# instadeepai/FrameDiPT

Measured on AMD Instinct MI355X. Metric: residue*diffusion-steps/sec, higher is better.
Workload: dtype fp16

## Files before the change

### framedipt_amd/csrc/model.hip

```cpp
#include <math.h>
#include <string.h>

#include <vector>

#include "common.hpp"
#include "kernels.hpp"

struct LinW { long w, b; int out, in; };
struct LNW { long g, b; int d; };
#define FD_MAX_BLOCKS 8
#define FD_MAX_TL 4
struct TfLayer { LinW inp, outp, l1, l2; LNW n1, n2; };
struct BlockW {
  long head_w;
  LinW q, kv, qp, kvp, lb, dz, out, rbf;
  LNW ipa_ln;
  LinW skip;
  TfLayer tf[FD_MAX_TL];
  LinW post, t1, t2, t3;
  LNW tln;
  LinW bb;
  LinW et_init, et1, et2, etf;
  LNW et_ln;
};
// ... 542 lines not shown
  w.pz = take(use_regpair(d) ? fd_pz_bytes(B, N) : 0);
  w.ee_tab = take(ee_table_static(d, B, N) ? fd_ee2_table_bytes(B, ee_table_max_rel(N), d->num_bins) : 0);
  w.ee_idx = take(ee_table_static(d, B, N) ? NN * 4 : 0);
  w.ee_lead = take((size_t)B * 4);
  w.total = o;
}

size_t fdipt_forward_workspace_bytes(const FdiptDims* dims, int B, int N) {
  if (!dims_ok(dims) || B <= 0 || N <= 0) return 0;
  Inventory iv;
  DLayout L;
  WS w;
  build_inventory(dims, iv);
  blob_walk(dims, iv, L);
  build_ws(dims, iv, L, B, N, w);
  return w.total;
}

}

enum { OP_ALL, OP_EMBED, OP_POINTS, OP_IPA, OP_ET };
struct OpSel {
  int kind = OP_ALL, block = 0;
  const float* node_in = nullptr;
  const void* z_in = nullptr;
  void* z_out = nullptr;
  float* node_out = nullptr;
  float* out = nullptr;
  float *qp = nullptr, *kp = nullptr, *vp = nullptr;
};

enum NodeForm { NF_GEMM, NF_ROWBLOCK, NF_ROWS16 };
enum SkipAt { SKIP_PER_BLOCK, SKIP_EMBED16, SKIP_SPLITK };
enum OutProj { OUT_GEMM, OUT_DEDICATED, OUT_SPLITK_SPLIT };
enum NodeRows { NR_PROJ, NR_POINTS, NR_LAUNCH };
enum SeqAttn { SEQ_FUSED, SEQ_BF16, SEQ_F32, SEQ_GENERIC };
enum PostAt { POST_TAIL, POST_CHAIN, POST_GEMM };
enum EtKind { ET_GEMM, ET_CHAIN, ET_ET3, ET_ET4 };
enum EtRows { ETR_IMAGES, ETR_ROWS, ETR_FOLDED };
struct ForwardPlan {
  int op;
  bool bf, fused_node;
  NodeForm embed, tail, transition, torsion;
  SkipAt skip;
  OutProj outproj;
  int slices;
// ... 112 lines not shown
  size_t NN;
  const float* res_mask = a->res_mask;
  float* F(size_t off) const { return (float*)(W + off); }
  FdStep step() const { return FdStep{a->step_cursor, a->frame_rows, a->state_ring}; }
  const void* WM(const LinW& l) const { return p.bf ? (const void*)((const half_t*)(D + L.h16_base) + l.w) : (const void*)(P + l.w); }
  int lin(const LinW& l, const float* A, int lda, const float* res, int ldr, const float* rm, int relu, float* out, int ldo) const {
    return fd_linear(op_precision(d), R, l.out, l.in, A, lda, WM(l), l.in, P + l.b, res, ldr, rm, relu, out, ldo, st);
  }
  int lin32(const LinW& l, const float* A, int lda, float* out, int ldo) const {
    return fd_linear(FDIPT_PREC_F32, R, l.out, l.in, A, lda, P + l.w, l.in, P + l.b, nullptr, 0, nullptr, 0, out, ldo, st);
  }
  int d2d(void* dst, const void* src, size_t bytes) const {
    return hipMemcpyAsync(dst, src, bytes, hipMemcpyDeviceToDevice, st) == hipSuccess ? FDIPT_OK : FDIPT_ELAUNCH;
  }
  int inner(int b, int slot, const float* src, int ld, int cols) const {
    if (!a->trace_inner) return FDIPT_OK;
    float* dst = a->trace_inner + ((size_t)(b * 4 + slot) * R) * iv.d_t;
    return hipMemcpy2DAsync(dst, (size_t)iv.d_t * 4, src, (size_t)ld * 4, (size_t)cols * 4, R, hipMemcpyDeviceToDevice, st) == hipSuccess
               ? FDIPT_OK : FDIPT_ELAUNCH;
  }
  bool first_block(int b) const { return b == 0 || p.op != OP_ALL; }
  bool bias_ready(int b) const { return p.op == OP_ALL && (b == 0 ? p.ee_bias : (p.et == ET_ET3 || p.et == ET_ET4) && p.et_bias); }
  bool fold_et_rows(int b) const { return p.et_rows == ETR_FOLDED && b < d->num_blocks - 1; }
  L2Warm warm_of(int b, WarmOf next, int l = 0) const {
    const DBlock& db = L.blk[b];
    const int cs = d->c_s, dt = iv.d_t;
    const unsigned tb = (unsigned)fd_chain_image_bytes(cs, cs);
    switch (next) {
      case WARM_QKV: {
        const unsigned n = (unsigned)fd_chain_image_bytes(3 * dt, dt);
        return L2Warm{{D + db.ch.inp[l], D + db.lo.inp[l], nullptr}, {n, n, 0}};
      }
      case WARM_TAIL: {
        if (p.tail == NF_ROWS16) return L2Warm{{D + db.lo.o16[l][0], D + db.lo.o16[l][1], nullptr}, {db.lo.tail16_run[l], db.lo.tail16_run[l], 0}};
        const unsigned wimg = (unsigned)fd_chain_image_bytes(dt, dt);
        return L2Warm{{D + db.ch.outp[l], D + db.ch.l1[l], D + db.ch.l2[l]}, {wimg, wimg, wimg}};
      }
      case WARM_POST: return L2Warm{{D + db.ch.post, nullptr, nullptr}, {(unsigned)fd_chain_image_bytes(cs, dt), 0, 0}};
      case WARM_TRANSITION:
        if (p.transition == NF_ROWS16) return L2Warm{{D + db.lo.tr16[0][0], D + db.lo.tr16[0][1], nullptr}, {db.lo.tr16_run, db.lo.tr16_run, 0}};
        return L2Warm{{D + db.ch.t1, D + db.ch.t2, D + db.lo.t1}, {tb, db.ch.t23_run, db.lo.t_run}};
      case WARM_TRANSITION32:
        return L2Warm{{D + db.ch.t1, D + db.ch.t2, D + db.ch.t3}, {tb, tb, tb}};
      case WARM_ET_ROWS: {
        const unsigned ei = (unsigned)fd_chain_image_bytes(iv.cb, cs), r4 = (unsigned)fd_chain_image_bytes(2 * (iv.hid + d->c_z), iv.cb);
        return L2Warm{{D + db.ch.et_init, D + db.ch.r4w, D + db.lo.et_init}, {ei, r4, db.lo.et_run}};
      }
      case WARM_ET_FOLDED:
        return L2Warm{{D + db.lo.ei16[0], D + db.lo.ei16[1], nullptr}, {db.lo.et16_run, db.lo.et16_run, 0}};
      case WARM_TORSION:
        if (p.torsion == NF_ROWS16) return L2Warm{{D + L.tor16[0][0], D + L.tor16[0][1], nullptr}, {L.tor16_run, L.tor16_run, 0}};
        return L2Warm{{D + L.ch_tor1, D + L.ch_tor2, D + L.lo_tor1}, {tb, tb, L.lo_tor_run}};
    }
    return L2Warm{};
  }
  int embed_stage() const {
    const int cs = d->c_s, cz = d->c_z;
    RC(fd_build_feats(B, N, d->use_aatype, d->index_embed, a->aatype, a->t_emb, a->t_emb_eps, a->fixed_mask, a->idx_emb, F(w.node_feat),
                      L.kn_pad, F(w.pte), L.d1_pad, p.feats_fused ? a->rigids_t : nullptr, a->res_mask, d->coordinate_scaling, F(w.quat),
                      F(w.trans), F(w.dmask), (const float*)(D + L.w1i), (const float*)(D + L.w1j), (const float*)(D + L.b1), cz,
                      p.feats_fused ? F(w.pi) : nullptr, F(w.pj), step(), st));
    if (p.embed == NF_GEMM) {
      RC(fd_linear(op_precision(d), R, cs, L.kn_pad, F(w.node_feat), L.kn_pad, D + L.ne0_pad, L.kn_pad, P + iv.ne0.b, nullptr, 0, nullptr, 1,
                   F(w.h_a), cs, st));
      RC(lin(iv.ne2, F(w.h_a), cs, nullptr, 0, nullptr, 1, F(w.h_b), cs));
      RC(lin(iv.ne4, F(w.h_b), cs, nullptr, 0, nullptr, 0, F(w.h_a), cs));
      RC(fd_layernorm(R, cs, F(w.h_a), cs, nullptr, 0, P + iv.neln.g, P + iv.neln.b, a->res_mask, F(w.node0), cs, st));
    } else {
      const bool r16 = p.embed == NF_ROWS16;
      RowBlockArgs r;
      r.M = R; r.in = F(w.node_feat); r.ld_in = L.kn_pad;
      r.w0 = D + (r16 ? L.ne16[0][0] : L.ch_ne0); r.w1 = D + (r16 ? L.ne16[1][0] : L.ch_ne2); r.w2 = D + (r16 ? L.ne16[2][0] : L.ch_ne4);
      r.w0l = D + (r16 ? L.ne16[0][1] : L.lo_ne0); r.w1l = D + (r16 ? L.ne16[1][1] : L.lo_ne2); r.w2l = D + (r16 ? L.ne16[2][1] : L.lo_ne4);
      r.b0 = P + iv.ne0.b; r.b1 = P + iv.ne2.b; r.b2 = P + iv.ne4.b;
      r.gamma = P + iv.neln.g; r.beta = P + iv.neln.b; r.rowmask_post = a->res_mask; r.out = F(w.node0); r.ld_out = cs;
      if (p.skip == SKIP_EMBED16) {
        r.w3 = D + L.skip16[0]; r.w3l = D + L.skip16[1]; r.b3 = (const float*)(D + L.skip_b);
        r.out2 = F(w.skip_all); r.ld_out2 = d->num_blocks * d->c_skip;
        r.warm = L2Warm{{r.w0, r.w0l, r.w3}, {L.ne16_run, L.ne16_run, L.skip16_run}};
      }
      if (r16) RC(fd_node_embed16(r, L.kn_pad, st));
      else RC(fd_rowblock(L.kn_pad == 72 ? FD_RB_NODE_EMBED_72 : FD_RB_NODE_EMBED_88, r, st));
    }
    if (!p.feats_fused) {
      RC(fd_linear(FDIPT_PREC_F32, R, cz, L.d1_pad, F(w.pte), L.d1_pad, D + L.w1i, L.d1_pad, (const float*)(D + L.b1), nullptr, 0,
                   nullptr, 0, F(w.pi), cz, st));
      RC(fd_linear(FDIPT_PREC_F32, R, cz, L.d1_pad, F(w.pte), L.d1_pad, D + L.w1j, L.d1_pad, nullptr, nullptr, 0, nullptr, 0,
                   F(w.pj), cz, st));
    }
    EdgeEmbedArgs ea;
    ea.B = B; ea.N = N; ea.n_rel = a->n_rel; ea.rel_off = a->rel_off; ea.num_bins = d->num_bins;
    ea.pi = F(w.pi); ea.pj = F(w.pj); ea.rtab = (const float*)setup; ea.dtab = d->num_bins > 0 ? (const float*)(D + L.dtab) : nullptr;
    ea.edges = d->num_bins > 0 ? (const float*)(D + L.edges) : nullptr; ea.seq_idx = a->seq_idx; ea.sc_ca = a->sc_ca_t;
    ea.w2 = WM(iv.ee2); ea.w3 = WM(iv.ee4); ea.b2 = P + iv.ee2.b; ea.b3 = P + iv.ee4.b;
    ea.gamma = P + iv.eeln.g; ea.beta = P + iv.eeln.b; ea.res_mask = a->res_mask; ea.z_out = W + w.z;
    ea.trace = a->trace_edge; ea.reserve_cus = a->reserve_cus;
    ea.wb_img = p.ee_bias ? D + L.blk[0].wb_img4 : nullptr; ea.bb = (const float*)(D + L.blk[0].bb); ea.bias_out = F(w.bias); ea.H = d->no_heads;
    if (p.pz) {
      ea.wdz_img = D + L.blk[0].wdz_imgp; ea.wdz_img_lo = D + L.blk[0].wdz_imgp_lo; ea.bdz = P + iv.blk[0].dz.b; ea.pz_out = (half_t*)(W + w.pz);
    }
    if (p.ee_table) {
      ea.fixed_mask = a->fixed_mask; ea.table = W + w.ee_tab; ea.row_idx = (int32_t*)(W + w.ee_idx); ea.leaders = (int32_t*)(W + w.ee_lead);
      ea.rel_lead = (const int32_t*)((const char*)setup + setup_rel_lead(d, B, a->n_rel));
      RC(fd_edge_embed2_leaders(ea, st));
      RC(fd_edge_embed2_table(ea, D + (p.x ? L.ee2x : L.ee2), st, p.x));
      ea.pz_out = nullptr;
      RC(fd_edge_embed2_spread(ea, st, 0));
    } else if (p.regpair) RC(fd_edge_embed2(ea, D + (p.x ? L.ee2x : L.ee2), st, p.x));
    else RC(fd_edge_embed(op_precision(d), cz, ea, st));
    return FDIPT_OK;
  }
  int ipa_project(int b, const float* node) const {
    const DBlock& db = L.blk[b];
    const int cs = d->c_s, H = d->no_heads, C = d->c_hidden, Pq = d->no_qk_points, Pv = d->no_v_points, PT = iv.proj_out - 3 * H * C;
    PointsArgs pa;
    pa.B = B; pa.N = N; pa.H = H; pa.Pq = Pq; pa.Pv = Pv; pa.quat = F(w.quat); pa.trans = F(w.trans);
    pa.qp = F(w.qp); pa.kp = F(w.kp); pa.vp = F(w.vp); pa.rot = F(w.rot);
    pa.vpt = p.vpt ? (unsigned short*)(W + w.vpt) : nullptr; pa.Np = Np;
    if (!p.a3) {
      RC(fd_linear(op_precision(d), R, iv.proj_out, cs, node, cs, D + db.wproj, cs, (const float*)(D + db.bproj), nullptr, 0,
                   nullptr, 0, F(w.proj), iv.proj_out, st));
      pa.proj = F(w.proj); pa.ld = iv.proj_out; pa.q_off = 3 * H * C; pa.kv_off = 3 * H * C + 3 * H * Pq;
      return fd_points(pa, st);
    }
    pa.kpf = (unsigned short*)(W + w.kpf); pa.gamma = (const float*)(D + db.gamma); pa.res_mask = a->res_mask;
    ProjArgs pj;
    pj.B = B; pj.N = N; pj.H = H; pj.C = C; pj.K = cs; pj.PT = PT; pj.Np = Np; pj.A = node; pj.lda = cs;
    pj.W = D + db.wproj; pj.bias = (const float*)(D + db.bproj); pj.qscale = sqrtf(1.0f / (3.0f * (float)C));
    pj.Qb = (half_t*)(W + w.qb); pj.Kb = (half_t*)(W + w.kb); pj.Vt = (half_t*)(W + w.vt); pj.pts = F(w.pts);
    pj.zero_pads = first_block(b);
    pj.W_img = proj_image(d) ? D + db.wproj_img : nullptr;
    pj.W_img_lo = pj.W_img && p.fused_node ? D + db.wproj_img_lo : nullptr;
    if (p.merged) { pj.merged = 1; pj.W_img = D + db.wproj2_img; pj.W_img_lo = D + db.wproj2_img_lo; pj.bias = (const float*)(D + db.bproj2); }
    if (p.proj_pts) {
      pj.pts_img = 1; pj.W_img = D + db.wproj2p_img; pj.W_img_lo = D + db.wproj2p_img_lo; pj.bias = (const float*)(D + db.bproj2p);
      pj.PT = fd_ipa_proj2_points_cols(H, C) - H * C;
      pj.quat = pa.quat; pj.trans = pa.trans; pj.gamma = pa.gamma; pj.res_mask = pa.res_mask; pj.rot = pa.rot; pj.qp = pa.qp;
      pj.kpf = pa.kpf; pj.vpt = pa.vpt;
    }
    if (p.vt_lo && p.node_rows == NR_PROJ) pj.Vt_lo = (half_t*)(W + w.vt_lo);
    const size_t vpt_bytes = (size_t)B * H * 96 * Np * 2;
    bool vpt_zero = pa.vpt && first_block(b);
    if (p.proj2) {
      const bool key_pads = Np > N && p.node_rows == NR_PROJ;
      if (pj.zero_pads && p.init_fused) {
        SeqInitExtra sx = {vpt_zero ? W + w.vpt : nullptr, vpt_zero ? (long)(vpt_bytes >> 4) : 0L, key_pads ? (void*)pj.Kb : nullptr,
                           (void*)pj.Vt, (long)B * H, C, (void*)pj.Vt_lo};
        RC(fd_seq_images_init(B, N, d->tfmr_heads, a->res_mask, W + w.seqimg, sx, st, p.stream));
        vpt_zero = false;
      } else if (pj.zero_pads && (key_pads || vpt_zero)) {
        ProjArgs pz = pj; pz.W_img = nullptr;
        if (p.node_rows != NR_PROJ) pz.Np = pz.N;
        RC(fd_ipa_proj_zero_pads(pz, vpt_zero ? W + w.vpt : nullptr, vpt_zero ? vpt_bytes : 0, st));
        vpt_zero = false;
      }
      RC(fd_ipa_proj2(pj, st));
      half_t* vt_lo = (half_t*)(W + w.vt_lo);
      if (p.node_rows == NR_POINTS) { pa.node = node; pa.ld_node = cs; pa.nKb = pj.Kb; pa.nVt = pj.Vt; pa.nVt_lo = vt_lo; }
      if (p.node_rows == NR_LAUNCH) RC(fd_node_images(B, N, Np, node, cs, pj.Kb, pj.Vt, vt_lo, st));
    } else RC(fd_ipa_proj(pj, st));
    if (vpt_zero && hipMemsetAsync(W + w.vpt, 0, vpt_bytes, st) != hipSuccess) return FDIPT_ELAUNCH;
    pa.proj = F(w.pts); pa.ld = PT; pa.q_off = 0; pa.kv_off = 3 * H * Pq;
    if (!p.proj_pts) RC(fd_points(pa, st));
    return FDIPT_OK;
  }
  int ipa_attend(int b) const {
    const DBlock& db = L.blk[b];
    const int cz = d->c_z, H = d->no_heads, C = d->c_hidden, Pv = d->no_v_points, feat = iv.feat_dim;
    OPairArgs oa;
    oa.B = B; oa.N = N; oa.H = H; oa.CZ = cz; oa.CD = cz / 4; oa.z = W + w.z; oa.probs = F(w.probs); oa.probs_h16 = nullptr;
    oa.probs_np = 0; oa.out_h16 = nullptr; oa.wdz = (const float*)(D + db.wdz_t); oa.wdz_img = p.bf && dz_images(d) ? D + db.wdz_img : nullptr;
// ... 255 lines not shown
    if (!setup || !a->fixed_mask || (!a->sc_ca_t && d->num_bins > 0) || !a->seq_idx || !a->idx_emb || !a->t_emb) return FDIPT_EINVAL;
    if (d->use_aatype && (!a->aatype || !a->t_emb_eps)) return FDIPT_EINVAL;
  }
  if (op.kind == OP_ALL && (!a->rigids_t || !a->gt_psi || !a->t || !a->so3_sigma || !a->psi || !a->rot_score || !a->trans_score ||
                            !a->rigids))
    return FDIPT_EINVAL;
  if ((op.kind == OP_POINTS || op.kind == OP_IPA) && !a->rigids_t) return FDIPT_EINVAL;
  if (!FdStep{a->step_cursor, a->frame_rows, a->state_ring}.valid()) return FDIPT_EINVAL;
  if (op.kind != OP_ALL && op.kind != OP_EMBED && (op.block < 0 || op.block >= d->num_blocks - (op.kind == OP_ET ? 1 : 0))) return FDIPT_EINVAL;
  Inventory iv;
  DLayout L;
  WS w;
  build_inventory(d, iv);
  blob_walk(d, iv, L);
  const int B = a->B, N = a->N, R = B * N;
  build_ws(d, iv, L, B, N, w);
  if (workspace_bytes < w.total) return FDIPT_ESIZE;
  if ((long)B * N * N > 2000000000L / 1) return FDIPT_ESIZE;
  const ForwardPlan p = plan_forward(d, iv, L, B, N, op.kind, a->n_rel, a->trace_edge != nullptr, a->pair_embed != 0);
  if (p.refused) return FDIPT_EINVAL;
  const Fwd f = {d, iv, L, w, p, P, (const char*)derived, (char*)workspace, setup, a, (hipStream_t)stream, B, N, R, (N + 31) / 32 * 32, (size_t)R * N};
  if (a->trace_inner && (p.fused_node || p.outproj != OUT_GEMM)) return FDIPT_EINVAL;
  const size_t node_bytes = (size_t)R * d->c_s * 4, z_bytes = f.NN * d->c_z * L.esz;
  if (op.kind == OP_ALL || op.kind == OP_EMBED) RC(f.embed_stage());
  if (op.kind == OP_EMBED) {
    if (op.node_out) RC(f.d2d(op.node_out, f.F(w.node0), node_bytes));
    if (op.z_out) RC(f.d2d(op.z_out, f.W + w.z, z_bytes));
    return FDIPT_OK;
  }
  if (a->trace_node && op.kind == OP_ALL) RC(f.d2d(a->trace_node, f.F(w.node0), node_bytes));
  if (!p.feats_fused && a->rigids_t)
    RC(fd_split_rigids(R, a->rigids_t, d->coordinate_scaling, a->res_mask, a->fixed_mask ? a->fixed_mask : a->res_mask, f.F(w.quat),
                       f.F(w.trans), f.F(w.dmask), f.step(), f.st));
  if (op.kind != OP_ALL) {
    if (!op.node_in) return FDIPT_EINVAL;
    RC(f.d2d(f.F(w.node), op.node_in, node_bytes));
    if (op.kind != OP_POINTS) {
      if (!op.z_in) return FDIPT_EINVAL;
      RC(f.d2d(f.W + w.z, op.z_in, z_bytes));
    }
    const int b = op.block;
    if (op.kind == OP_ET) {
      RC(f.edge_transition_stage(b, f.F(w.node)));
      if (!op.z_out) return FDIPT_EINVAL;
      return f.d2d(op.z_out, f.W + w.z, z_bytes);
    }
// ... 39 lines not shown
  build_inventory(d, iv);
  blob_walk(d, iv, L);
  const ForwardPlan p = plan_forward(d, iv, L, B, N, OP_ALL, n_rel, false, false);
  return p.ee_table && !p.refused ? (int64_t)n_rel * (d->num_bins + 1) : 0;
}

int fdipt_embed_table_leaders(const FdiptDims* d, const void* workspace, int B, int N, int n_rel, int32_t* out_dev) {
  if (!workspace || !out_dev || fdipt_embed_table_rows(d, B, N, n_rel) <= 0) return FDIPT_EINVAL;
  Inventory iv;
  DLayout L;
  WS w;
  build_inventory(d, iv);
  blob_walk(d, iv, L);
  build_ws(d, iv, L, B, N, w);
  if (hipDeviceSynchronize() != hipSuccess) return FDIPT_ELAUNCH;
  return hipMemcpy(out_dev, (const char*)workspace + w.ee_lead, (size_t)B * 4, hipMemcpyDeviceToDevice) == hipSuccess ? FDIPT_OK : FDIPT_ELAUNCH;
}

int fdipt_score_forward(const FdiptDims* d, const float* P, const void* derived, const void* setup,
                        const FdiptForwardArgs* a, void* workspace, size_t workspace_bytes, fdipt_stream_t stream) {
  return forward_impl(d, P, derived, setup, a, workspace, workspace_bytes, stream, OpSel{});
}

int fdipt_edge_embed_fwd(const FdiptDims* d, const float* P, const void* derived, const void* setup, const FdiptForwardArgs* a,
                         float* node_out, void* z_out, void* workspace, size_t workspace_bytes, fdipt_stream_t stream) {
  OpSel op;
  op.kind = OP_EMBED; op.node_out = node_out; op.z_out = z_out;
  return forward_impl(d, P, derived, setup, a, workspace, workspace_bytes, stream, op);
}

static FdiptForwardArgs op_args(int B, int N, const float* rigids_t, const float* res_mask) {
  FdiptForwardArgs a;
  memset(&a, 0, sizeof(a));
  a.B = B; a.N = N; a.rigids_t = rigids_t; a.res_mask = res_mask;
  return a;
}
int fdipt_ipa_project_points(const FdiptDims* d, const float* P, const void* derived, int block, int B, int N, const float* node,
                             const float* rigids, const float* res_mask, float* q_pts, float* k_pts, float* v_pts,
                             void* workspace, size_t workspace_bytes, fdipt_stream_t stream) {
  OpSel op;
  op.kind = OP_POINTS; op.block = block; op.node_in = node; op.qp = q_pts; op.kp = k_pts; op.vp = v_pts;
  const FdiptForwardArgs a = op_args(B, N, rigids, res_mask);
  return forward_impl(d, P, derived, nullptr, &a, workspace, workspace_bytes, stream, op);
}
int fdipt_ipa_attention_fwd(const FdiptDims* d, const float* P, const void* derived, int block, int B, int N, const float* node,
                            const void* z, const float* rigids, const float* res_mask, float* out, void* workspace,
// ... 34 lines not shown
```

### framedipt_amd/inference.py

```python
from __future__ import annotations

import ctypes as C

import numpy as np
import torch

from . import _lib, gpu_guard
from . import noise as noise_mod
from .model.score_network import preprocess_aatype


def draw_noise_tape(diffuser, n_steps: int, B: int, N: int):
    z_rot = np.zeros((n_steps, B, N, 3))
    z_trans = np.zeros((n_steps, B, N, 3))
    for s in range(n_steps):
        if diffuser._diffuse_rot:
            z_rot[s] = np.random.normal(size=(B, N, 3))
        if diffuser._diffuse_trans:
            z_trans[s] = np.random.normal(size=(B, N, 3))
    return z_rot, z_trans


def kept_steps(num_t: int, keep="all") -> np.ndarray:
    num_t = int(num_t)
# ... 27 lines not shown
    _lib.check(lib.fdipt_backbone_atoms(n, _lib.ptr(t7), _lib.ptr(rot), _lib.ptr(trans), _lib.ptr(psi), _lib.ptr(aatype),
                                        _lib.ptr(net.bb_tables), _lib.ptr(atom37), None, _lib.stream_ptr()),
               "backbone_atoms")


def get_atom_positions_from_rigids(model, rigids, psi_torsions, aatype=None) -> np.ndarray:
    t7 = rigids.to_tensor_7() if hasattr(rigids, "to_tensor_7") else rigids
    dev = model.device
    with torch.cuda.device(dev):
        t7 = t7.to(device=dev, dtype=torch.float32).contiguous()
        psi = psi_torsions.to(device=dev, dtype=torch.float32).contiguous()
        aa = None if aatype is None else aatype.to(device=dev, dtype=torch.int32).contiguous()
        atom37 = torch.empty(t7.shape[:-1] + (37, 3), dtype=torch.float32, device=dev)
        _backbone(model, int(np.prod(t7.shape[:-1])), t7, None, None, psi, aa, atom37)
        return atom37.cpu().numpy()


class ReverseLoop:

    GRAPH_CHUNK = 8

    def __init__(self, model, diffuser, data_init, num_t, min_t, center=True, aux_traj=False, self_condition=True,
                 noise_scale=1.0, embed_self_conditioning=True, inpainting=False, input_aatype=False, noise_tape=None, state=None,
                 graph=True, verify=0, noise="host", noise_keys=None, keep="all"):
        self.model, self.diffuser = model, diffuser
        self.keep = keep
        steps = kept_steps(num_t, keep)
        self.kept = keep != "all"
        keys = noise_mod.resolve(noise, noise_keys, noise_tape, int(data_init["rigids_t"].shape[0]))
        dev = self.dev = model.device
        gpu_guard.check(dev, what="inference_fn")
        self.verify, self.verified = int(verify or 0), 0
        rig0 = data_init["rigids_t"]
        _lib.require_cuda(rig0, "inference_fn")
        if rig0.dim() == 2:
            raise ValueError("rigids_t needs a leading batch dimension")
        B, N = self.B, self.N = rig0.shape[0], rig0.shape[1]
        f32 = lambda x: x.to(device=dev, dtype=torch.float32).contiguous().clone()
        self.res_mask, self.fixed = f32(data_init["res_mask"]), f32(data_init["fixed_mask"])
        self.fixed_mask = (self.fixed * self.res_mask).contiguous()
        self.diffuse_mask = ((1 - self.fixed) * self.res_mask).contiguous()
        self._inpainting, self._input_aatype = inpainting, input_aatype
        self.aatype, self.net_aatype, same = _aatype_views(model, data_init, self.fixed, inpainting, input_aatype, dev)
        self.bb0_from_forward = same
        self.gt_tors = data_init["torsion_angles_sin_cos"]
        self.gt_psi = f32(self.gt_tors[..., 2, :])
        self.st = state if state is not None else model.batch_state(data_init["seq_idx"])
        self.num_t, self.min_t, self.dt = num_t, min_t, 1 / num_t
        self.center, self.aux_traj, self.noise_scale = center, aux_traj, noise_scale
        self.self_condition, self.embed_sc = self_condition, embed_self_conditioning
        self.reverse_steps = np.linspace(min_t, 1.0, num_t)[::-1]
        n_noisy = self.n_noisy = int(np.sum(self.reverse_steps > min_t))
        t32, temb, sig = model.step_scalars(self.reverse_steps)
        with torch.cuda.device(dev):
            self.t_all = torch.as_tensor(np.repeat(t32[:, None], B, 1), device=dev)
            self.temb_all = torch.as_tensor(np.repeat(temb[:, None, :], B, 1), device=dev)
            self.sig_all = torch.as_tensor(np.repeat(sig[:, None], B, 1), device=dev)
            self.t_tab = torch.as_tensor(np.ascontiguousarray(self.reverse_steps, dtype=np.float64), device=dev)
            so3 = diffuser._so3_diffuser
            self.tab_all = self.omega_edges = None
            if so3.use_cached_score:
                rows = so3.score_table_rows(t32)
                self.tab_all = torch.as_tensor(np.repeat(rows[:, None, :], B, 1), device=dev)
                self.omega_edges = torch.as_tensor(so3.omega_edges, device=dev)
            self.z_rot = self.z_trans = self.noise_keys = None
            if keys is not None:
                self.noise_keys = noise_mod.keys_tensor(keys, dev)
            else:
                if noise_tape is None:
                    noise_tape = draw_noise_tape(diffuser, n_noisy, B, N)
                self.z_rot = torch.as_tensor(np.ascontiguousarray(noise_tape[0], dtype=np.float64), device=dev)
                self.z_trans = torch.as_tensor(np.ascontiguousarray(noise_tape[1], dtype=np.float64), device=dev)
            self.sc_ca = f32(data_init["sc_ca_t"])
            self.kept_steps, n_rows = steps, len(steps)
            self.frame_rows = self.kept_rigids = None
            self._row_of = None
# ... 12 lines not shown
            self.trans_traj = torch.empty(n_rows, B, N, 3, device=dev) if aux_traj else None
            self.cursor = torch.zeros(2, dtype=torch.int32, device=dev)
        self.graph = bool(graph) and n_noisy >= 3 and (keys is not None or (self.z_rot.shape[0] >= n_noisy and self.z_trans.shape[0] >= n_noisy))
        self._cursor_host = 0
        self._g1 = self._gn = None
        self.capture_seconds = 0.0
        self.captures = 0

    @property
    def rigids_t(self):
        return self._x(self._next)

    _next = 0

    def _x(self, k):
        return self.rigid_traj[k & 1] if self.kept else self.rigid_traj[k]

    def _row(self, k):
        if not self.kept:
            return k
        r = int(self._row_of[k])
        return None if r < 0 else r

    def _fwd(self, k, want_atoms, sc_update):
        row = self._row(k)
        want_atoms = want_atoms and row is not None
        direct = want_atoms and self.bb0_from_forward
        self.st.score_table = None if self.tab_all is None else self.tab_all[k]
        self.st.omega_edges = self.omega_edges
        self.st.forward(self._x(k), self.res_mask, self.fixed, self.sc_ca, self.net_aatype, self.gt_psi, self.t_all[k],
                        self.temb_all[k], self.sig_all[k], direct, ca_out=self.sc_ca if sc_update else None,
                        atom37_out=self.bb0_traj[row] if direct else None)
        if want_atoms and not direct:
            _backbone(self.model, self.B * self.N, self.st.rigids, None, None, self.st.psi, self.aatype, self.bb0_traj[row])

    def prime(self):
        if self.embed_sc and self.self_condition:
            with torch.cuda.device(self.dev):
                self._fwd(0, False, True)

    def _verify_forward(self, k):
        st = self.st
        self.st.score_table = None if self.tab_all is None else self.tab_all[k]
        self.st.omega_edges = self.omega_edges
        st.forward(self._x(k), self.res_mask, self.fixed, self.sc_ca, self.net_aatype, self.gt_psi, self.t_all[k],
                   self.temb_all[k], self.sig_all[k], False)
        return [x.clone() for x in (st.rigids, st.psi, st.rot_score, st.trans_score)]

    def _step_eager(self, k):
        st, t, n = self.st, self.reverse_steps[k], self.B * self.N
        first = self._verify_forward(k) if self.verify and k % self.verify == 0 else None
        self._fwd(k, self.aux_traj, self.embed_sc and t > self.min_t)
        if first is not None:
            for name, a, b in zip(("rigids", "psi", "rot_score", "trans_score"), first, (st.rigids, st.psi, st.rot_score, st.trans_score)):
                if not torch.equal(a, b):
                    raise _lib.FdiptError(f"verify: two runs of the forward of step {k} differ in `{name}` (max |diff| "
                                          f"{float((a - b).abs().max()):.3e}): results on this GPU are not reproducible — is another "
                                          "compute process using it? (DESIGN.md section 6)")
            self.verified += 1
        nxt, row = self._x(k + 1), self._row(k)
        if t > self.min_t:
            dev_noise = self.noise_keys is not None
            self.diffuser.reverse_device(self._x(k), st.rot_score, st.trans_score, self.diffuse_mask,
                                         None if dev_noise else self.z_rot[k], None if dev_noise else self.z_trans[k], t, self.dt,
                                         self.center, self.noise_scale, rigids_out=nxt, noise_keys=self.noise_keys, step=k,
                                         atoms=(st.psi, self.aatype, self.model.bb_tables, self.prot_traj[row]) if row is not None else None,
                                         traj=(st.rigids, self.fixed_mask, self.trans_traj[row]) if self.aux_traj and row is not None else None)
        else:
            nxt.copy_(st.rigids)
            _backbone(self.model, n, nxt, None, None, st.psi, self.aatype, self.prot_traj[row])
            if self.aux_traj:
                self.trans_traj[row] = self.diffuse_mask[..., None] * st.rigids[..., 4:] + self.fixed_mask[..., None] * nxt[..., 4:]
        if self.kept_rigids is not None and row is not None:
            self.kept_rigids[row].copy_(nxt)

    def _enqueue_indexed(self):
        lib, st, d = _lib.load(), self.st, self.diffuser
        direct = self.aux_traj and self.bb0_from_forward
        st.score_table, st.omega_edges = self.tab_all, self.omega_edges
        st.forward(self.rigid_traj, self.res_mask, self.fixed, self.sc_ca, self.net_aatype, self.gt_psi, self.t_all, self.temb_all,
                   self.sig_all, direct, ca_out=self.sc_ca if self.embed_sc else None, atom37_out=self.bb0_traj if direct else None,
                   step_cursor=self.cursor, frame_rows=self.frame_rows, state_ring=self.kept)
        if self.aux_traj and not direct:
            args = [self.B * self.N, _lib.ptr(st.rigids), _lib.ptr(st.psi), _lib.ptr(self.aatype), _lib.ptr(self.model.bb_tables),
                    _lib.ptr(self.bb0_traj), _lib.ptr(self.cursor)]
            if self.kept:
                _lib.check(lib.fdipt_backbone_atoms_kept(*args, _lib.ptr(self.frame_rows), _lib.stream_ptr()), "backbone_atoms_kept")
            else:
                _lib.check(lib.fdipt_backbone_atoms_indexed(*args, _lib.stream_ptr()), "backbone_atoms_indexed")
        so3, r3 = d._so3_diffuser, d._r3_diffuser
        a = _lib.ReverseIndexed()
        a.B, a.N = self.B, self.N
        for name, tns in (("rigid_traj", self.rigid_traj), ("rot_score", st.rot_score), ("trans_score", st.trans_score),
                          ("diffuse_mask", self.diffuse_mask), ("z_rot", self.z_rot), ("z_trans", self.z_trans), ("t_table", self.t_tab),
                          ("psi", st.psi), ("aatype", self.aatype), ("bb_tables", self.model.bb_tables), ("prot_traj", self.prot_traj),
                          ("pred_rigids", st.rigids if self.aux_traj else None), ("traj_fixed_mask", self.fixed_mask if self.aux_traj else None),
                          ("trans_traj", self.trans_traj), ("step_cursor", self.cursor), ("frame_rows", self.frame_rows),
                          ("kept_rigids", self.kept_rigids)):
            setattr(a, name, _lib.ptr(tns))
        a.state_ring = int(self.kept)
        a.dt, a.noise_scale = float(self.dt), float(self.noise_scale)
        a.center, a.diffuse_rot, a.diffuse_trans = int(bool(self.center)), int(bool(d._diffuse_rot)), int(bool(d._diffuse_trans))
        a.so3_min_sigma, a.so3_max_sigma, a.r3_min_b, a.r3_max_b = so3.min_sigma, so3.max_sigma, r3.min_b, r3.max_b
        a.coordinate_scaling = r3._r3_conf.coordinate_scaling
        if self.noise_keys is not None:
# ... 24 lines not shown
            self.cursor[:1].fill_(k)
            self._cursor_host = k

    _WARM: set = set()

    def _warm_key(self):
        return (str(self.dev), bytes(self.model.dims), self.B, self.N, bool(self.aux_traj), bool(self.bb0_from_forward),
                bool(self._inpainting), self.tab_all is not None, bool(self.embed_sc), bool(self.self_condition),
                self.noise_keys is not None, bool(self.kept))

    def prepare(self):
        if self.graph and self._warm_key() in self._WARM:
            with torch.cuda.device(self.dev):
                if self._g1 is None:
                    self._g1 = self.capture_step_graph(1)
                if self._gn is None and self.GRAPH_CHUNK > 1 and self.n_noisy >= 2 * self.GRAPH_CHUNK:
                    self._gn = self.capture_step_graph(self.GRAPH_CHUNK)
        return self

    def _advance(self, k, n, eager=False):
        self._set_cursor(k)
        if (self._g1 is not None or self._gn is not None) and self._captured_weights != getattr(self.model, "weights_version", 0):
            self._g1 = self._gn = None
        if eager or self._warm_key() not in self._WARM:
            for _ in range(n):
                self._enqueue_indexed()
            self._WARM.add(self._warm_key())
        elif n > 1 and n == self.GRAPH_CHUNK:
            if self._gn is None:
                self._gn = self.capture_step_graph(n)
            self._gn.replay()
        else:
            if self._g1 is None:
                self._g1 = self.capture_step_graph(1)
            for _ in range(n):
                self._g1.replay()
        self._cursor_host = k + n

    def step(self, k, eager=False):
        with torch.cuda.device(self.dev):
            if self.graph and k < self.n_noisy and not (self.verify and k % self.verify == 0):
                self._advance(k, 1, eager)
            else:
                self._step_eager(k)
        self._next = k + 1

# ... 47 lines not shown
        if self.diffuser._so3_diffuser.use_cached_score != (self.tab_all is not None):
            raise ValueError("reset: so3.use_cached_score changed behind the loop: the score-table switch selects other launches")
        before = self._warm_key()
        with torch.cuda.device(dev):
            f32 = lambda x: x.to(device=dev, dtype=torch.float32).contiguous()
            fixed = f32(data_init["fixed_mask"])
            aatype, net_aatype, same = _aatype_views(self.model, data_init, fixed, self._inpainting, self._input_aatype, dev)
            if same != self.bb0_from_forward or (aatype is None) != (self.aatype is None) or (net_aatype is None) != (self.net_aatype is None):
                raise ValueError("reset: this batch changes who builds the rigid_0_traj rows (bb0_from_forward / the aatype views): the captured "
                                 "launch sequence does not fit it; construct a new loop")
            seq_idx = data_init["seq_idx"]
            if tuple(seq_idx.shape) != (self.B, self.N):
                raise ValueError(f"reset: seq_idx of shape {tuple(seq_idx.shape)}, the loop holds B, N = {self.B}, {self.N}")
            keys = tape = None
            if self.noise_keys is not None:
                keys = noise_mod.keys_tensor(noise_mod.resolve("device", noise_keys, noise_tape, self.B), dev)
            else:
                if noise_tape is None:
                    noise_tape = draw_noise_tape(self.diffuser, self.n_noisy, self.B, self.N)
                tape = [torch.as_tensor(np.ascontiguousarray(z, dtype=np.float64)) for z in noise_tape]
                for dst, z in zip((self.z_rot, self.z_trans), tape):
                    if tuple(z.shape) != tuple(dst.shape):
                        raise ValueError(f"reset: noise tape of shape {tuple(z.shape)}, the loop's is {tuple(dst.shape)}")
            if getattr(self.model, "_state", None) is self.st:
                self.model._state = self.model._state_key = None
            if keys is not None:
                self.noise_keys.copy_(keys)
            else:
                self.z_rot.copy_(tape[0])
                self.z_trans.copy_(tape[1])
            self.res_mask.copy_(f32(data_init["res_mask"]))
            self.fixed.copy_(fixed)
            torch.mul(self.fixed, self.res_mask, out=self.fixed_mask)
            torch.mul(1 - self.fixed, self.res_mask, out=self.diffuse_mask)
            if aatype is not None:
                self.aatype.copy_(aatype)
            if net_aatype is not None:
                self.net_aatype.copy_(net_aatype)
            self.gt_tors = data_init["torsion_angles_sin_cos"]
            self.gt_psi.copy_(f32(self.gt_tors[..., 2, :]))
            self.sc_ca.copy_(f32(data_init["sc_ca_t"]))
            self.rigid_traj[0].copy_(rig0.to(device=dev, dtype=torch.float32))
            if not self.st.refresh(seq_idx):
                self._g1 = self._gn = None
            self.cursor.zero_()
        self._cursor_host, self._next, self.verified = 0, 0, 0
# ... 164 lines not shown
```

### framedipt_amd/model/score_network.py

```python
from __future__ import annotations

import ctypes as C
from collections import OrderedDict

import numpy as np
import torch

from .. import _lib, embedding, residue_tables, weights


PRECISIONS = {"fp32": _lib.PREC_F32, "f32": _lib.PREC_F32, "fp16": _lib.PREC_F16, "f16": _lib.PREC_F16,
              "fp16x": _lib.PREC_F16X, "f16x": _lib.PREC_F16X,
              "bf16": _lib.PREC_BF16}


def dims_from_conf(model_conf, diffuser_conf, inpainting: bool, precision: int, kernel_flags: int = 0) -> _lib.Dims:
    i, e = model_conf.ipa, model_conf.embed
    num_bins = e.num_bins if e.embed_self_conditioning else 0
    return _lib.Dims(i.c_s, i.c_z, i.c_hidden, i.c_skip, i.no_heads, i.no_qk_points, i.no_v_points,
                     i.seq_tfmr_num_heads, i.seq_tfmr_num_layers, i.num_blocks, e.index_embed_size, num_bins,
                     int(bool(inpainting or model_conf.input_aatype)), precision, kernel_flags, float(e.min_bin), float(e.max_bin),
                     float(i.coordinate_scaling), float(diffuser_conf.r3.min_b), float(diffuser_conf.r3.max_b))


# ... 55 lines not shown
    def refresh(self, seq_idx: torch.Tensor) -> bool:
        if tuple(seq_idx.shape) != (self.B, self.N):
            raise ValueError(f"refresh: seq_idx of shape {tuple(seq_idx.shape)}, the state holds B, N = {self.B}, {self.N}")
        lib, net, dev = _lib.load(), self.net, self.net.device
        sidx = seq_idx.detach().cpu().numpy().astype(np.int64)
        if np.array_equal(sidx, self._sidx):
            return True
        self._sidx = sidx
        E, d = net.dims.index_embed, net.dims
        with torch.cuda.device(dev):
            self.seq_idx.copy_(torch.as_tensor(sidx.astype(np.int32)))
            self.idx_emb.copy_(torch.as_tensor(embedding.get_index_embedding(sidx, E)))
            rng = int(sidx.max() - sidx.min())
            if rng == self.rel_off:
                return True
            self.rel_off, self.n_rel = rng, 2 * rng + 1
            rel = np.arange(self.n_rel) - rng
            rel_emb = torch.as_tensor(np.broadcast_to(embedding.get_index_embedding(rel, E)[None], (self.B, self.n_rel, E)).copy(), device=dev)
            self.setup = torch.empty(lib.fdipt_setup_bytes(C.byref(d), self.B, self.N, self.n_rel), dtype=torch.uint8, device=dev)
            _lib.check(lib.fdipt_sample_setup(C.byref(d), _lib.ptr(net.params), _lib.ptr(net.derived), self.B, self.N, self.n_rel,
                                              _lib.ptr(rel_emb), _lib.ptr(self.setup), _lib.stream_ptr()), "sample_setup")
        return False

    def forward(self, rigids_t, res_mask, fixed_mask, sc_ca_t, aatype, gt_psi, t_dev, t_emb_dev, sigma_dev,
                want_atoms: bool = True, ca_out=None, atom37_out=None, step_cursor=None, frame_rows=None, state_ring=False):
        lib = _lib.load()
        net = self.net
        a = _lib.ForwardArgs()
        a.B, a.N, a.n_rel, a.rel_off = self.B, self.N, self.n_rel, self.rel_off
        for name, tns in (("rigids_t", rigids_t), ("res_mask", res_mask), ("fixed_mask", fixed_mask), ("sc_ca_t", sc_ca_t),
                          ("seq_idx", self.seq_idx), ("idx_emb", self.idx_emb), ("aatype", aatype), ("gt_psi", gt_psi),
                          ("t", t_dev), ("t_emb", t_emb_dev), ("t_emb_eps", self.t_emb_eps), ("so3_sigma", sigma_dev),
                          ("bb_tables", net.bb_tables), ("psi", self.psi), ("rot_score", self.rot_score),
                          ("trans_score", self.trans_score), ("rigids", self.rigids),
                          ("atom37", (self.atom37 if atom37_out is None else atom37_out) if want_atoms else None), ("atom14", self.atom14 if want_atoms else None),
                          ("trace_node", self.trace_node), ("trace_edge", self.trace_edge), ("trace_inner", self.trace_inner),
                          ("ca_out", ca_out)):
            setattr(a, name, _lib.ptr(tns))
        if self.ev_start is not None:
            a.ev_start, a.ev_stop = self.ev_start, self.ev_stop
        a.reserve_cus = self.reserve_cus
        a.pair_embed = self.pair_embed
        a.step_cursor = _lib.ptr(step_cursor)
        if step_cursor is not None:
            a.frame_rows, a.state_ring = _lib.ptr(frame_rows), int(bool(state_ring))
        a.clock_out = _lib.ptr(self.clock_out)
        if self.score_table is not None:
            a.so3_score_table, a.so3_omega_edges = _lib.ptr(self.score_table), _lib.ptr(self.omega_edges)
            a.so3_num_omega = int(self.score_table.shape[-1])
        _lib.check(lib.fdipt_score_forward(C.byref(net.dims), _lib.ptr(net.params), _lib.ptr(net.derived),
                                           _lib.ptr(self.setup), C.byref(a), _lib.ptr(self.ws), self.ws_bytes,
                                           _lib.stream_ptr()), "score_forward")


class ScoreNetwork:
    def __init__(self, model_conf, diffuser, inpainting: bool = False, precision: str = "fp32", device=None,
                 kernel_flags: int = 0):
        self._model_conf = model_conf
# ... 119 lines not shown
```

### include/fdipt.h

```cpp
#ifndef FDIPT_H
#define FDIPT_H

#include <stddef.h>
#include <stdint.h>

#ifdef __cplusplus
extern "C" {
#endif

#define FDIPT_OK 0
#define FDIPT_EINVAL (-1)
#define FDIPT_ELAUNCH (-2)
#define FDIPT_ESIZE (-3)

#define FDIPT_PREC_F32 0
#define FDIPT_PREC_BF16 1
#define FDIPT_PREC_F16 2
#define FDIPT_PREC_F16X 3

#define FDIPT_KF_ET3 1
#define FDIPT_KF_GENERIC_PAIR 2
#define FDIPT_KF_GENERIC_ATTN 4
#define FDIPT_KF_UNFUSED_NODE 8
#define FDIPT_KF_UNFOLDED 16
// ... 19 lines not shown
  int32_t num_blocks;
  int32_t index_embed;
  int32_t num_bins;
  int32_t use_aatype;
  int32_t precision;
  int32_t kernel_flags;
  float min_bin;
  float max_bin;
  float coordinate_scaling;
  float r3_min_b;
  float r3_max_b;
} FdiptDims;

int fdipt_param_count(const FdiptDims* dims);
int64_t fdipt_param_offset(const FdiptDims* dims, int index);

size_t fdipt_derived_bytes(const FdiptDims* dims);
int fdipt_model_prepare(const FdiptDims* dims, const float* params_f32, void* derived, fdipt_stream_t stream);

size_t fdipt_setup_bytes(const FdiptDims* dims, int B, int N, int n_rel);
int fdipt_sample_setup(const FdiptDims* dims, const float* params_f32, const void* derived, int B, int N, int n_rel,
                       const float* rel_emb, void* setup, fdipt_stream_t stream);

typedef struct FdiptForwardArgs {
  int32_t B, N, n_rel, rel_off;
  const float* rigids_t;
  const float* res_mask;
  const float* fixed_mask;
  const float* sc_ca_t;
  const int32_t* seq_idx;
  const float* idx_emb;
  const int32_t* aatype;
  const float* gt_psi;
  const float* t;
  const float* t_emb;
  const float* t_emb_eps;
  const double* so3_sigma;
  const void* bb_tables;
  float* psi;
  double* rot_score;
  float* trans_score;
  float* rigids;
  float* atom37;
  float* atom14;
  float* trace_node;
  float* trace_edge;
  float* trace_inner;
  void** ev_start;
  void** ev_stop;
  float* ca_out;
  int32_t reserve_cus;
  int32_t pair_embed;
  unsigned long long* clock_out;
  const double* so3_score_table;
  const double* so3_omega_edges;
  int32_t so3_num_omega;
  const int32_t* step_cursor;
  const int32_t* frame_rows;
  int32_t state_ring;
} FdiptForwardArgs;

size_t fdipt_forward_workspace_bytes(const FdiptDims* dims, int B, int N);
int64_t fdipt_embed_table_rows(const FdiptDims* dims, int B, int N, int n_rel);
int fdipt_embed_table_leaders(const FdiptDims* dims, const void* workspace, int B, int N, int n_rel, int32_t* out_dev);
int fdipt_score_forward(const FdiptDims* dims, const float* params_f32, const void* derived, const void* setup,
                        const FdiptForwardArgs* args, void* workspace, size_t workspace_bytes, fdipt_stream_t stream);

int fdipt_edge_embed_fwd(const FdiptDims* dims, const float* params_f32, const void* derived, const void* setup,
                         const FdiptForwardArgs* args, float* node_out, void* z_out, void* workspace, size_t workspace_bytes,
                         fdipt_stream_t stream);
int fdipt_ipa_project_points(const FdiptDims* dims, const float* params_f32, const void* derived, int block, int B, int N,
                             const float* node, const float* rigids, const float* res_mask, float* q_pts, float* k_pts,
                             float* v_pts, void* workspace, size_t workspace_bytes, fdipt_stream_t stream);
int fdipt_ipa_attention_fwd(const FdiptDims* dims, const float* params_f32, const void* derived, int block, int B, int N,
                            const float* node, const void* z, const float* rigids, const float* res_mask, float* out,
                            void* workspace, size_t workspace_bytes, fdipt_stream_t stream);
int fdipt_edge_transition_fwd(const FdiptDims* dims, const float* params_f32, const void* derived, int block, int B, int N,
                              const float* node, const float* res_mask, const void* z_in, void* z_out, void* workspace,
                              size_t workspace_bytes, fdipt_stream_t stream);

int fdipt_se3_reverse_step(int B, int N, const float* rigids_t, const double* rot_score, const float* trans_score,
                           const float* diffuse_mask , const double* z_rot, const double* z_trans,
                           double t, double dt, double noise_scale, int center, int diffuse_rot, int diffuse_trans,
                           double so3_min_sigma, double so3_max_sigma, double r3_min_b, double r3_max_b,
                           double coordinate_scaling, float* rigids_out , float* out_rot ,
                           fdipt_stream_t stream);
int fdipt_se3_reverse_step_atoms(int B, int N, const float* rigids_t, const double* rot_score, const float* trans_score,
                                 const float* diffuse_mask, const double* z_rot, const double* z_trans, double t, double dt,
                                 double noise_scale, int center, int diffuse_rot, int diffuse_trans, double so3_min_sigma,
// ... 606 lines not shown
```

Measured before the change: 1.231 million.

## Precompute step-invariant edge-table leaders and sequence image pads once per sample

Result: no change. 1.238 million (median of 6 runs) (+0.5%).

```diff
diff --git a/framedipt_amd/csrc/model.hip b/framedipt_amd/csrc/model.hip
--- a/framedipt_amd/csrc/model.hip
+++ b/framedipt_amd/csrc/model.hip
@@ -588,6 +588,7 @@
 enum { OP_ALL, OP_EMBED, OP_POINTS, OP_IPA, OP_ET };
 struct OpSel {
   int kind = OP_ALL, block = 0;
+  bool constants = false;
   const float* node_in = nullptr;
   const void* z_in = nullptr;
   void* z_out = nullptr;
@@ -746,6 +747,11 @@
   bool first_block(int b) const { return b == 0 || p.op != OP_ALL; }
   bool bias_ready(int b) const { return p.op == OP_ALL && (b == 0 ? p.ee_bias : (p.et == ET_ET3 || p.et == ET_ET4) && p.et_bias); }
   bool fold_et_rows(int b) const { return p.et_rows == ETR_FOLDED && b < d->num_blocks - 1; }
+  bool constants_plan() const {
+    return p.op == OP_ALL && p.ee_table && p.a3 && p.seq == SEQ_FUSED && p.init_fused && !p.stream && p.proj_pts && p.node_rows == NR_PROJ && p.vt_lo;
+  }
+  bool pads_kept() const { return constants_plan() && (a->step_constants & FDIPT_SC_PADS); }
+  bool leaders_kept() const { return constants_plan() && (a->step_constants & FDIPT_SC_LEADERS); }
   L2Warm warm_of(int b, WarmOf next, int l = 0) const {
     const DBlock& db = L.blk[b];
     const int cs = d->c_s, dt = iv.d_t;
@@ -778,13 +784,14 @@
     }
     return L2Warm{};
   }
-  int embed_stage() const {
+  int embed_stage(bool leaders_only = false) const {
     const int cs = d->c_s, cz = d->c_z;
     RC(fd_build_feats(B, N, d->use_aatype, d->index_embed, a->aatype, a->t_emb, a->t_emb_eps, a->fixed_mask, a->idx_emb, F(w.node_feat),
                       L.kn_pad, F(w.pte), L.d1_pad, p.feats_fused ? a->rigids_t : nullptr, a->res_mask, d->coordinate_scaling, F(w.quat),
                       F(w.trans), F(w.dmask), (const float*)(D + L.w1i), (const float*)(D + L.w1j), (const float*)(D + L.b1), cz,
                       p.feats_fused ? F(w.pi) : nullptr, F(w.pj), step(), st));
-    if (p.embed == NF_GEMM) {
+    if (leaders_only) {
+    } else if (p.embed == NF_GEMM) {
       RC(fd_linear(op_precision(d), R, cs, L.kn_pad, F(w.node_feat), L.kn_pad, D + L.ne0_pad, L.kn_pad, P + iv.ne0.b, nullptr, 0, nullptr, 1,
                    F(w.h_a), cs, st));
       RC(lin(iv.ne2, F(w.h_a), cs, nullptr, 0, nullptr, 1, F(w.h_b), cs));
@@ -826,13 +833,26 @@
     if (p.ee_table) {
       ea.fixed_mask = a->fixed_mask; ea.table = W + w.ee_tab; ea.row_idx = (int32_t*)(W + w.ee_idx); ea.leaders = (int32_t*)(W + w.ee_lead);
       ea.rel_lead = (const int32_t*)((const char*)setup + setup_rel_lead(d, B, a->n_rel));
-      RC(fd_edge_embed2_leaders(ea, st));
+      if (leaders_only || !leaders_kept()) RC(fd_edge_embed2_leaders(ea, st));
+      if (leaders_only) return FDIPT_OK;
       RC(fd_edge_embed2_table(ea, D + (p.x ? L.ee2x : L.ee2), st, p.x));
       ea.pz_out = nullptr;
       RC(fd_edge_embed2_spread(ea, st, 0));
     } else if (p.regpair) RC(fd_edge_embed2(ea, D + (p.x ? L.ee2x : L.ee2), st, p.x));
     else RC(fd_edge_embed(op_precision(d), cz, ea, st));
     return FDIPT_OK;
+  }
+  int images_init(bool vpt_zero, bool key_pads, bool vt_lo) const {
+    const int H = d->no_heads;
+    const size_t vpt_bytes = (size_t)B * H * 96 * Np * 2;
+    SeqInitExtra sx = {vpt_zero ? W + w.vpt : nullptr, vpt_zero ? (long)(vpt_bytes >> 4) : 0L, key_pads ? (void*)(W + w.kb) : nullptr,
+                       (void*)(W + w.vt), (long)B * H, d->c_hidden, vt_lo ? (void*)(W + w.vt_lo) : nullptr};
+    return fd_seq_images_init(B, N, d->tfmr_heads, a->res_mask, W + w.seqimg, sx, st, p.stream);
+  }
+  int step_constants_stage() const {
+    if (!constants_plan()) return FDIPT_EINVAL;
+    RC(embed_stage(true));
+    return images_init(true, Np > N, true);
   }
   int ipa_project(int b, const float* node) const {
     const DBlock& db = L.blk[b];
@@ -867,10 +887,10 @@
     bool vpt_zero = pa.vpt && first_block(b);
     if (p.proj2) {
       const bool key_pads = Np > N && p.node_rows == NR_PROJ;
-      if (pj.zero_pads && p.init_fused) {
-        SeqInitExtra sx = {vpt_zero ? W + w.vpt : nullptr, vpt_zero ? (long)(vpt_bytes >> 4) : 0L, key_pads ? (void*)pj.Kb : nullptr,
-                           (void*)pj.Vt, (long)B * H, C, (void*)pj.Vt_lo};
-        RC(fd_seq_images_init(B, N, d->tfmr_heads, a->res_mask, W + w.seqimg, sx, st, p.stream));
+      if (pj.zero_pads && pads_kept()) {
+        vpt_zero = false;
+      } else if (pj.zero_pads && p.init_fused) {
+        RC(images_init(vpt_zero, key_pads, pj.Vt_lo != nullptr));
         vpt_zero = false;
       } else if (pj.zero_pads && (key_pads || vpt_zero)) {
         ProjArgs pz = pj; pz.W_img = nullptr;
@@ -1172,6 +1192,7 @@
   const Fwd f = {d, iv, L, w, p, P, (const char*)derived, (char*)workspace, setup, a, (hipStream_t)stream, B, N, R, (N + 31) / 32 * 32, (size_t)R * N};
   if (a->trace_inner && (p.fused_node || p.outproj != OUT_GEMM)) return FDIPT_EINVAL;
   const size_t node_bytes = (size_t)R * d->c_s * 4, z_bytes = f.NN * d->c_z * L.esz;
+  if (op.constants) return f.step_constants_stage();
   if (op.kind == OP_ALL || op.kind == OP_EMBED) RC(f.embed_stage());
   if (op.kind == OP_EMBED) {
     if (op.node_out) RC(f.d2d(op.node_out, f.F(w.node0), node_bytes));
@@ -1257,6 +1278,26 @@
   return forward_impl(d, P, derived, setup, a, workspace, workspace_bytes, stream, OpSel{});
 }
 
+int fdipt_forward_step_constants(const FdiptDims* d, const float* P, const void* derived, const void* setup,
+                                 const FdiptForwardArgs* a, void* workspace, size_t workspace_bytes, fdipt_stream_t stream) {
+  OpSel op;
+  op.constants = true;
+  return forward_impl(d, P, derived, setup, a, workspace, workspace_bytes, stream, op);
+}
+
+int fdipt_forward_image_offsets(const FdiptDims* d, int B, int N, int64_t* offsets_host) {
+  if (!dims_ok(d) || B <= 0 || N <= 0 || !offsets_host) return FDIPT_EINVAL;
+  Inventory iv;
+  DLayout L;
+  WS w;
+  build_inventory(d, iv);
+  blob_walk(d, iv, L);
+  build_ws(d, iv, L, B, N, w);
+  const size_t off[5] = {w.seqimg, w.kb, w.vt, w.vt_lo, w.vpt};
+  for (int i = 0; i < 5; ++i) offsets_host[i] = (int64_t)off[i];
+  return FDIPT_OK;
+}
+
 int fdipt_edge_embed_fwd(const FdiptDims* d, const float* P, const void* derived, const void* setup, const FdiptForwardArgs* a,
                          float* node_out, void* z_out, void* workspace, size_t workspace_bytes, fdipt_stream_t stream) {
   OpSel op;
diff --git a/framedipt_amd/inference.py b/framedipt_amd/inference.py
--- a/framedipt_amd/inference.py
+++ b/framedipt_amd/inference.py
@@ -73,7 +73,7 @@
 
     def __init__(self, model, diffuser, data_init, num_t, min_t, center=True, aux_traj=False, self_condition=True,
                  noise_scale=1.0, embed_self_conditioning=True, inpainting=False, input_aatype=False, noise_tape=None, state=None,
-                 graph=True, verify=0, noise="host", noise_keys=None, keep="all"):
+                 graph=True, verify=0, noise="host", noise_keys=None, keep="all", step_constants=True):
         self.model, self.diffuser = model, diffuser
         self.keep = keep
         steps = kept_steps(num_t, keep)
@@ -103,6 +103,9 @@
         self.reverse_steps = np.linspace(min_t, 1.0, num_t)[::-1]
         n_noisy = self.n_noisy = int(np.sum(self.reverse_steps > min_t))
         t32, temb, sig = model.step_scalars(self.reverse_steps)
+        self._t_host, self._temb_host = np.repeat(t32[:, None], B, 1), np.repeat(temb[:, None, :], B, 1)
+        bits = (_lib.SC_PADS | _lib.SC_LEADERS) if step_constants is True else int(step_constants or 0)
+        self.step_constants = bits if self.st.step_constants_supported() and self.st.uniform_t(self._t_host, self._temb_host) else 0
         with torch.cuda.device(dev):
             self.t_all = torch.as_tensor(np.repeat(t32[:, None], B, 1), device=dev)
             self.temb_all = torch.as_tensor(np.repeat(temb[:, None, :], B, 1), device=dev)
@@ -161,29 +164,55 @@
         r = int(self._row_of[k])
         return None if r < 0 else r
 
+    @property
+    def constants_token(self):
+        tok = self.__dict__.get("_constants_token")
+        if tok is None:
+            tok = self.__dict__["_constants_token"] = object()
+        return tok
+
+    def _ensure_constants(self):
+        if self.step_constants and self.st.constants_owner is not self.constants_token:
+            self.st.write_step_constants(self.constants_token, self.rigid_traj[0], self.res_mask, self.fixed, self.sc_ca, self.net_aatype, self.gt_psi,
+                                         self.t_all[0], self.temb_all[0], self.sig_all[0], self._t_host, self._temb_host)
+
+    def _drop_constants(self):
+        if self.st.constants_owner is self.constants_token:
+            self.st.constants_owner = None
+
+    def _constants(self, k=None):
+        if not self.step_constants:
+            return {}
+        t, temb = (self._t_host, self._temb_host) if k is None else (self._t_host[k], self._temb_host[k])
+        return dict(constants_owner=self.constants_token, constants=self.step_constants, t_host=t, t_emb_host=temb)
+
     def _fwd(self, k, want_atoms, sc_update):
         row = self._row(k)
         want_atoms = want_atoms and row is not None
         direct = want_atoms and self.bb0_from_forward
         self.st.score_table = None if self.tab_all is None else self.tab_all[k]
         self.st.omega_edges = self.omega_edges
+        self._ensure_constants()
         self.st.forward(self._x(k), self.res_mask, self.fixed, self.sc_ca, self.net_aatype, self.gt_psi, self.t_all[k],
                         self.temb_all[k], self.sig_all[k], direct, ca_out=self.sc_ca if sc_update else None,
-                        atom37_out=self.bb0_traj[row] if direct else None)
+                        atom37_out=self.bb0_traj[row] if direct else None,
+                        **self._constants(k))
         if want_atoms and not direct:
             _backbone(self.model, self.B * self.N, self.st.rigids, None, None, self.st.psi, self.aatype, self.bb0_traj[row])
 
     def prime(self):
-        if self.embed_sc and self.self_condition:
-            with torch.cuda.device(self.dev):
+        with torch.cuda.device(self.dev):
+            self._ensure_constants()
+            if self.embed_sc and self.self_condition:
                 self._fwd(0, False, True)
 
     def _verify_forward(self, k):
         st = self.st
         self.st.score_table = None if self.tab_all is None else self.tab_all[k]
         self.st.omega_edges = self.omega_edges
+        self._ensure_constants()
         st.forward(self._x(k), self.res_mask, self.fixed, self.sc_ca, self.net_aatype, self.gt_psi, self.t_all[k],
-                   self.temb_all[k], self.sig_all[k], False)
+                   self.temb_all[k], self.sig_all[k], False, **self._constants(k))
         return [x.clone() for x in (st.rigids, st.psi, st.rot_score, st.trans_score)]
 
     def _step_eager(self, k):
@@ -219,7 +248,7 @@
         st.score_table, st.omega_edges = self.tab_all, self.omega_edges
         st.forward(self.rigid_traj, self.res_mask, self.fixed, self.sc_ca, self.net_aatype, self.gt_psi, self.t_all, self.temb_all,
                    self.sig_all, direct, ca_out=self.sc_ca if self.embed_sc else None, atom37_out=self.bb0_traj if direct else None,
-                   step_cursor=self.cursor, frame_rows=self.frame_rows, state_ring=self.kept)
+                   step_cursor=self.cursor, frame_rows=self.frame_rows, state_ring=self.kept, **self._constants())
         if self.aux_traj and not direct:
             args = [self.B * self.N, _lib.ptr(st.rigids), _lib.ptr(st.psi), _lib.ptr(self.aatype), _lib.ptr(self.model.bb_tables),
                     _lib.ptr(self.bb0_traj), _lib.ptr(self.cursor)]
@@ -290,6 +319,7 @@
         self._set_cursor(k)
         if (self._g1 is not None or self._gn is not None) and self._captured_weights != getattr(self.model, "weights_version", 0):
             self._g1 = self._gn = None
+        self._ensure_constants()
         if eager or self._warm_key() not in self._WARM:
             for _ in range(n):
                 self._enqueue_indexed()
@@ -383,6 +413,7 @@
                 for dst, z in zip((self.z_rot, self.z_trans), tape):
                     if tuple(z.shape) != tuple(dst.shape):
                         raise ValueError(f"reset: noise tape of shape {tuple(z.shape)}, the loop's is {tuple(dst.shape)}")
+            self._drop_constants()
             if getattr(self.model, "_state", None) is self.st:
                 self.model._state = self.model._state_key = None
             if keys is not None:
diff --git a/framedipt_amd/model/score_network.py b/framedipt_amd/model/score_network.py
--- a/framedipt_amd/model/score_network.py
+++ b/framedipt_amd/model/score_network.py
@@ -101,18 +101,67 @@
                                               _lib.ptr(rel_emb), _lib.ptr(self.setup), _lib.stream_ptr()), "sample_setup")
         return False
 
-    def forward(self, rigids_t, res_mask, fixed_mask, sc_ca_t, aatype, gt_psi, t_dev, t_emb_dev, sigma_dev,
-                want_atoms: bool = True, ca_out=None, atom37_out=None, step_cursor=None, frame_rows=None, state_ring=False):
-        lib = _lib.load()
-        net = self.net
+    def _args(self, rigids_t, res_mask, fixed_mask, sc_ca_t, aatype, gt_psi, t_dev, t_emb_dev, sigma_dev):
         a = _lib.ForwardArgs()
         a.B, a.N, a.n_rel, a.rel_off = self.B, self.N, self.n_rel, self.rel_off
         for name, tns in (("rigids_t", rigids_t), ("res_mask", res_mask), ("fixed_mask", fixed_mask), ("sc_ca_t", sc_ca_t),
                           ("seq_idx", self.seq_idx), ("idx_emb", self.idx_emb), ("aatype", aatype), ("gt_psi", gt_psi),
                           ("t", t_dev), ("t_emb", t_emb_dev), ("t_emb_eps", self.t_emb_eps), ("so3_sigma", sigma_dev),
-                          ("bb_tables", net.bb_tables), ("psi", self.psi), ("rot_score", self.rot_score),
-                          ("trans_score", self.trans_score), ("rigids", self.rigids),
-                          ("atom37", (self.atom37 if atom37_out is None else atom37_out) if want_atoms else None), ("atom14", self.atom14 if want_atoms else None),
+                          ("bb_tables", self.net.bb_tables), ("psi", self.psi), ("rot_score", self.rot_score),
+                          ("trans_score", self.trans_score), ("rigids", self.rigids)):
+            setattr(a, name, _lib.ptr(tns))
+        return a
+
+    constants_owner = None
+
+    @staticmethod
+    def uniform_t(t_host, t_emb_host) -> bool:
+        t_host, t_emb_host = np.asarray(t_host), np.asarray(t_emb_host)
+        return bool(np.all(t_host == t_host[..., :1]) and np.all(t_emb_host == t_emb_host[..., :1, :]))
+
+    def step_constants_supported(self) -> bool:
+        if self.trace_edge is not None or self.pair_embed:
+            return False
+        return _lib.load().fdipt_embed_table_rows(C.byref(self.net.dims), self.B, self.N, self.n_rel) > 0
+
+    def write_step_constants(self, owner, rigids_t, res_mask, fixed_mask, sc_ca_t, aatype, gt_psi, t_dev, t_emb_dev, sigma_dev,
+                             t_host, t_emb_host) -> bool:
+        self.constants_owner = None
+        if owner is None or not self.step_constants_supported() or not self.uniform_t(t_host, t_emb_host):
+            return False
+        a = self._args(rigids_t, res_mask, fixed_mask, sc_ca_t, aatype, gt_psi, t_dev, t_emb_dev, sigma_dev)
+        net = self.net
+        rc = _lib.load().fdipt_forward_step_constants(C.byref(net.dims), _lib.ptr(net.params), _lib.ptr(net.derived), _lib.ptr(self.setup),
+                                                      C.byref(a), _lib.ptr(self.ws), self.ws_bytes, _lib.stream_ptr())
+        if rc != _lib.EINVAL:
+            _lib.check(rc, "forward_step_constants")
+        self.constants_owner = owner
+        return rc == 0
+
+    def forward(self, rigids_t, res_mask, fixed_mask, sc_ca_t, aatype, gt_psi, t_dev, t_emb_dev, sigma_dev,
+                want_atoms: bool = True, ca_out=None, atom37_out=None, step_cursor=None, frame_rows=None, state_ring=False,
+                constants_owner=None, constants=None, t_host=None, t_emb_host=None):
+        lib = _lib.load()
+        net = self.net
+        keep = 0
+        if constants_owner is not None:
+            if t_host is None or t_emb_host is None:
+                raise ValueError("constants_owner needs t_host and t_emb_host: one t per step is checked on the host")
+            seen = self.__dict__.get("_uniform_seen")
+            if seen is not None and seen[0] is t_host and seen[1] is t_emb_host:
+                pass
+            elif self.uniform_t(t_host, t_emb_host):
+                self._uniform_seen = (t_host, t_emb_host)
+            else:
+                raise _lib.FdiptError("forward with step constants: the samples of the batch are not at one t; call it without constants_owner")
+            if self.constants_owner is not constants_owner and not torch.cuda.is_current_stream_capturing():
+                raise _lib.FdiptError("forward with step constants: another call has used this state since write_step_constants")
+            keep = (_lib.SC_PADS | _lib.SC_LEADERS) if constants is None else int(constants) & (_lib.SC_PADS | _lib.SC_LEADERS)
+        if constants_owner is None:
+            self.constants_owner = None
+        a = self._args(rigids_t, res_mask, fixed_mask, sc_ca_t, aatype, gt_psi, t_dev, t_emb_dev, sigma_dev)
+        a.step_constants = keep
+        for name, tns in (("atom37", (self.atom37 if atom37_out is None else atom37_out) if want_atoms else None), ("atom14", self.atom14 if want_atoms else None),
                           ("trace_node", self.trace_node), ("trace_edge", self.trace_edge), ("trace_inner", self.trace_inner),
                           ("ca_out", ca_out)):
             setattr(a, name, _lib.ptr(tns))
diff --git a/include/fdipt.h b/include/fdipt.h
--- a/include/fdipt.h
+++ b/include/fdipt.h
@@ -65,6 +65,8 @@
 int fdipt_sample_setup(const FdiptDims* dims, const float* params_f32, const void* derived, int B, int N, int n_rel,
                        const float* rel_emb, void* setup, fdipt_stream_t stream);
 
+#define FDIPT_SC_PADS 1
+#define FDIPT_SC_LEADERS 2
 typedef struct FdiptForwardArgs {
   int32_t B, N, n_rel, rel_off;
   const float* rigids_t;
@@ -98,6 +100,7 @@
   const double* so3_score_table;
   const double* so3_omega_edges;
   int32_t so3_num_omega;
+  int32_t step_constants;
   const int32_t* step_cursor;
   const int32_t* frame_rows;
   int32_t state_ring;
@@ -108,6 +111,9 @@
 int fdipt_embed_table_leaders(const FdiptDims* dims, const void* workspace, int B, int N, int n_rel, int32_t* out_dev);
 int fdipt_score_forward(const FdiptDims* dims, const float* params_f32, const void* derived, const void* setup,
                         const FdiptForwardArgs* args, void* workspace, size_t workspace_bytes, fdipt_stream_t stream);
+int fdipt_forward_step_constants(const FdiptDims* dims, const float* params_f32, const void* derived, const void* setup,
+                                 const FdiptForwardArgs* args, void* workspace, size_t workspace_bytes, fdipt_stream_t stream);
+int fdipt_forward_image_offsets(const FdiptDims* dims, int B, int N, int64_t* offsets_host);
 
 int fdipt_edge_embed_fwd(const FdiptDims* dims, const float* params_f32, const void* derived, const void* setup,
                          const FdiptForwardArgs* args, float* node_out, void* z_out, void* workspace, size_t workspace_bytes,
```
